# GiorgiaAuroraAdorni/gansformer-reproducibility-challenge

Measured on NVIDIA H100. Metric: images/sec @256^2 synth (GANsformer generator forward, K=16 latents, 12 attention layers, batch 32/GPU), higher is better.
Workload: dtype tf32 (fp32 storage; wgmma tf32 attention and stride-1 3x3 convolutions (own kernels), TF32 cuDNN up-convolutions; value_fp32_convs = the same with fp32 cuDNN convolutions)

## Files before the change

gansformer-reproducibility-challenge_b200/_lib.py:

```python
from __future__ import annotations

import ctypes
from ctypes import c_int, c_int32, c_size_t, c_void_p, c_char_p, POINTER, byref
from typing import Optional

from ._build import LIB_PATH, build_extension

GF_OK = 0
NORM = {None: 0, "none": 0, "layer": 1, "instance": 2, "batch": 3}
INTEGRATION = {"mul": 0, "add": 1, "both": 2}
FLAG_FP32_EXACT = 1
FLAG_CENTROIDS_IN = 2
FLAG_TABLES_READY = 4
FLAG_IMG2LTNT = 8
FLAG_CENTROIDS_INIT = 16
PATH_NAMES = {0: "none", 1: "simt_fp32", 2: "wgmma_tf32"}

WEIGHT_FIELDS = ("wq", "bq", "wpq", "wk", "bk", "wpk", "wv", "bv", "wo", "bo", "pos_latent",
                 "wq2", "bq2", "wpq2", "wk2", "bk2", "wpk2", "wv2", "bv2", "wkc", "wcq", "wi2l", "bi2l")

EXPORTS = ("gf_attn_abi_version", "gf_last_error", "gf_attn_last_path", "gf_attn_folded_floats",
           "gf_attn_fold_weights", "gf_attn_workspace_bytes", "gf_attn_prologue", "gf_attn_simplex_fwd",
           "gf_attn_duplex_fwd", "gf_attn_norm_stats", "gf_attn_launch_count",
           "gf_attn_simplex_fwd_ex", "gf_attn_duplex_fwd_ex", "gf_attn_prologue_ex", "gf_attn_simplex_bwd", "gf_attn_last_centroid_path", "gf_attn_debug_layout",
           "gf_attn_prologue_batch", "gf_attn_tc_eligible", "gf_attn_simplex_bwd_ex", "gf_attn_dropout_mask",
           "gf_attn_centroid_stats", "gf_attn_centroid_bwd")
OPS_EXPORTS = ("gf_chan_scale_nhwc", "gf_blur_up_nhwc", "gf_upsample2x_nchw", "gf_bias_act_nhwc", "gf_demod_coef", "gf_torgb_nhwc", "gf_fir4_nhwc", "gf_blur_up_phases_nhwc", "gf_torgb_scale_nhwc", "gf_mapping_fwd", "gf_conv3x3_pack_weights", "gf_conv3x3_nhwc_tf32", "gf_demod_coef_batch")


class GfAttnDesc(ctypes.Structure):
    _fields_ = [(n, c_int32) for n in ("B", "H", "W", "C", "k", "D", "heads", "norm", "integration",
                                       "pos_dim", "duplex", "flags")]


class GfAttnWeights(ctypes.Structure):
    _fields_ = [(n, c_void_p) for n in WEIGHT_FIELDS]


class GfAttnPostop(ctypes.Structure):
    _fields_ = [("bias", c_void_p), ("noise", c_void_p), ("strength", c_void_p), ("noise_bstride", ctypes.c_longlong),
                ("act", c_int32), ("gain", ctypes.c_float), ("in_scale", c_void_p), ("post_scale", c_void_p),
                ("in_scale_ld", c_int32), ("post_scale_ld", c_int32),
                ("rgb_w", c_void_p), ("rgb_bias", c_void_p), ("rgb_out", c_void_p),
                ("att_dp", ctypes.c_float), ("dp_salt", ctypes.c_uint32), ("dp_state", c_void_p)]


_lib: Optional[ctypes.CDLL] = None


def load() -> ctypes.CDLL:
    global _lib
    if _lib is not None:
        return _lib
    import os
    alt = os.environ.get("GF_ATTN_LIB")
    if alt:
        lib = ctypes.CDLL(alt)
    else:
        try:
            build_extension()
        except Exception as e:
            if not LIB_PATH.exists():
                raise RuntimeError(f"libgf_attn.so is missing and could not be built: {e}") from e
        lib = ctypes.CDLL(str(LIB_PATH))
    lib.gf_attn_abi_version.restype = c_int
    lib.gf_last_error.restype = c_char_p
    lib.gf_attn_last_path.restype = c_int
    lib.gf_attn_folded_floats.argtypes = [POINTER(GfAttnDesc), POINTER(c_size_t)]
    lib.gf_attn_workspace_bytes.argtypes = [POINTER(GfAttnDesc), POINTER(c_size_t)]
    lib.gf_attn_fold_weights.argtypes = [POINTER(GfAttnDesc), POINTER(GfAttnWeights), c_void_p, c_void_p]
    lib.gf_attn_prologue.argtypes = [POINTER(GfAttnDesc), c_void_p, c_void_p, c_void_p, c_void_p]
    lib.gf_attn_simplex_fwd.argtypes = [POINTER(GfAttnDesc), c_void_p, c_void_p, c_void_p, c_void_p, c_void_p]
    lib.gf_attn_duplex_fwd.argtypes = [POINTER(GfAttnDesc), c_void_p, c_void_p, c_void_p, c_void_p, c_void_p,
                                       c_void_p, c_void_p, c_void_p]
    lib.gf_attn_norm_stats.argtypes = [POINTER(GfAttnDesc), c_void_p, c_void_p, c_void_p]
    lib.gf_attn_debug_layout.argtypes = [POINTER(GfAttnDesc), POINTER(ctypes.c_longlong), c_int]
    lib.gf_attn_prologue_ex.argtypes = [POINTER(GfAttnDesc), c_void_p, c_void_p, c_void_p, POINTER(GfAttnPostop), c_void_p]
    lib.gf_attn_simplex_fwd_ex.argtypes = [POINTER(GfAttnDesc), c_void_p, c_void_p, c_void_p, c_void_p, POINTER(GfAttnPostop), c_void_p]
    lib.gf_attn_duplex_fwd_ex.argtypes = [POINTER(GfAttnDesc), c_void_p, c_void_p, c_void_p, c_void_p, c_void_p,
                                          c_void_p, c_void_p, POINTER(GfAttnPostop), c_void_p]
    lib.gf_attn_prologue_batch.argtypes = [c_int, c_void_p, c_void_p, c_void_p, c_void_p, c_void_p, c_void_p]
    lib.gf_attn_simplex_bwd.argtypes = [POINTER(GfAttnDesc)] + [c_void_p] * 11
    lib.gf_attn_simplex_bwd_ex.argtypes = [POINTER(GfAttnDesc)] + [c_void_p] * 10 + [ctypes.c_float, ctypes.c_uint32, c_void_p, c_void_p, c_void_p]
    lib.gf_attn_dropout_mask.argtypes = [POINTER(GfAttnDesc), ctypes.c_float, ctypes.c_uint32, c_void_p, c_void_p, c_void_p]
    lib.gf_attn_centroid_stats.argtypes = [POINTER(GfAttnDesc)] + [c_void_p] * 8
    lib.gf_attn_centroid_bwd.argtypes = [POINTER(GfAttnDesc)] + [c_void_p] * 10
    lib.gf_chan_scale_nhwc.argtypes = [c_void_p, c_void_p, c_int, c_void_p, c_int, c_int, c_int, c_void_p]
    lib.gf_blur_up_nhwc.argtypes = [c_void_p, c_void_p, c_void_p, c_int, c_int, c_int, c_int, ctypes.c_float, c_void_p]
    lib.gf_upsample2x_nchw.argtypes = [c_void_p, c_void_p, c_void_p, c_int, c_int, c_int, c_int, c_void_p]
    lib.gf_bias_act_nhwc.argtypes = [c_void_p, c_void_p, c_void_p, c_void_p, c_void_p, ctypes.c_longlong, c_int, c_int, c_int,
                                     c_int, ctypes.c_float, c_void_p]
    lib.gf_demod_coef.argtypes = [c_void_p, c_int, c_void_p, c_void_p, c_int, c_int, c_int, ctypes.c_float, c_void_p]
    lib.gf_blur_up_phases_nhwc.argtypes = [c_void_p, c_void_p, c_void_p, c_void_p, c_void_p, c_void_p, c_int, c_int, c_int, c_int,
                                           ctypes.c_float, c_void_p]
    lib.gf_fir4_nhwc.argtypes = [c_void_p, c_void_p, c_int, c_int, c_int, c_int, c_int, ctypes.c_float, c_void_p]
    lib.gf_torgb_scale_nhwc.argtypes = [c_void_p, c_void_p, c_void_p, c_int, c_void_p, ctypes.c_float, c_void_p, c_void_p, c_int, c_void_p,
                                        c_int, c_int, c_int, c_void_p]
    lib.gf_mapping_fwd.argtypes = [c_void_p, c_void_p, c_void_p, c_void_p, ctypes.c_float, c_void_p, c_int, c_int, c_int, c_int, c_void_p]
    lib.gf_conv3x3_pack_weights.argtypes = [c_void_p, c_void_p, c_int, c_int, ctypes.c_float, c_void_p]
    lib.gf_conv3x3_nhwc_tf32.argtypes = [c_void_p, c_void_p, c_void_p, c_int, c_int, c_int, c_int, c_int, c_void_p]
    lib.gf_demod_coef_batch.argtypes = [c_void_p, c_int, c_int, ctypes.c_float, c_void_p]
    lib.gf_torgb_nhwc.argtypes = [c_void_p, c_void_p, c_void_p, c_int, c_void_p, ctypes.c_float, c_void_p, c_int, c_int, c_int, c_void_p]
    for name in OPS_EXPORTS:
        getattr(lib, name).restype = c_int
    for name in EXPORTS:
        fn = getattr(lib, name)
        if name not in ("gf_last_error", "gf_attn_launch_count"):
            fn.restype = c_int
    lib.gf_attn_launch_count.restype = ctypes.c_longlong
    lib.gf_attn_tc_eligible.argtypes = [POINTER(GfAttnDesc)]
    if lib.gf_attn_abi_version() != 2:
        raise RuntimeError("libgf_attn.so ABI version mismatch")
    _lib = lib
    return lib


class GfDemodJob(ctypes.Structure):
    _fields_ = [("styles", c_void_p), ("wsq", c_void_p), ("d", c_void_p), ("s_ld", ctypes.c_int32), ("O", ctypes.c_int32),
                ("I", ctypes.c_int32), ("pad_", ctypes.c_int32)]


DEMOD_MAX_JOBS = 32


def check(rc: int, what: str) -> None:
    if rc != GF_OK:
        msg = load().gf_last_error().decode("utf-8", "replace")
        raise RuntimeError(f"{what} failed (gf_status {rc}): {msg}")


def make_desc(B, H, W, C, k, D, *, heads=1, norm="layer", integration="mul", pos_dim=0, duplex=False, flags=0) -> GfAttnDesc:
    if norm not in NORM:
        raise ValueError(f"unknown norm {norm!r}")
    if integration not in INTEGRATION:
        raise ValueError(f"unknown integration {integration!r}")
    return GfAttnDesc(B, H, W, C, k, D, heads, NORM[norm], INTEGRATION[integration], pos_dim, int(duplex), flags)


def folded_floats(desc: GfAttnDesc) -> int:
    out = c_size_t(0)
    check(load().gf_attn_folded_floats(byref(desc), byref(out)), "gf_attn_folded_floats")
    return out.value


def workspace_bytes(desc: GfAttnDesc) -> int:
    out = c_size_t(0)
    check(load().gf_attn_workspace_bytes(byref(desc), byref(out)), "gf_attn_workspace_bytes")
    return out.value


def launch_count() -> int:
    return int(load().gf_attn_launch_count())


def last_centroid_path() -> str:
    return PATH_NAMES.get(load().gf_attn_last_centroid_path(), "?")


def last_path() -> str:
    return PATH_NAMES.get(load().gf_attn_last_path(), "?")
```

gansformer-reproducibility-challenge_b200/csrc/gf_conv.cu:

```cuda
#include <stdlib.h>
#include <string.h>
#include "gf_common.cuh"
#include "gf_tc_common.cuh"
#include "../../include/gf_ops.h"

namespace gf {
namespace cv {

using namespace tc;

constexpr int PH = 8, PW = 16;
constexpr int BK = 32;
constexpr int A_ROWS = (PH + 2) * PW;
constexpr int A_BYTES = A_ROWS * BK * 4;
constexpr int NUM_THREADS = 288;
constexpr int MAX_A = 3, MAX_W = 8;

struct Bars {
  uint64_t full_a[MAX_A], empty_a[MAX_A], full_w[MAX_W], empty_w[MAX_W];
};

struct Params {
  int B, H, W, Cin, Cout;
  int tiles_h, tiles_w, tiles_n;
// ... 39 lines not shown
    if (lane == 0) {
      int sa = 0, sw = 0; uint32_t pa = 0, pw_ = 0;
      for (long long t = blockIdx.x; t < P.total_tiles; t += gridDim.x) {
        int nt, pw, ph, b;
        decode(t, nt, pw, ph, b);
        const int h0 = ph * PH, w0 = pw * PW, n0 = nt * BN;
        for (int c0 = 0; c0 < P.Cin; c0 += BK) {
          for (int dx = 0; dx < 3; ++dx) {
            mbar_wait(smem_u32(&bars->empty_a[sa]), pa ^ 1u);
            const uint32_t fa = smem_u32(&bars->full_a[sa]);
            mbar_expect_tx(fa, (uint32_t)A_BYTES);
            tma_load_4d(s_a + (uint32_t)sa * A_BYTES, &tmX, fa, c0, w0 + dx - 1, h0 - 1, b);
            if (++sa == P.na) { sa = 0; pa ^= 1u; }
            for (int dy = 0; dy < 3; ++dy) {
              mbar_wait(smem_u32(&bars->empty_w[sw]), pw_ ^ 1u);
              const uint32_t fw = smem_u32(&bars->full_w[sw]);
              mbar_expect_tx(fw, (uint32_t)W_BYTES);
              tma_load_2d(s_w + (uint32_t)sw * W_BYTES, &tmW, fw, c0, (dy * 3 + dx) * P.Cout + n0);
              if (++sw == P.nw) { sw = 0; pw_ ^= 1u; }
            }
          }
        }
      }
    }
    return;
  }

  const int wg = warp >> 2;
  const int gid = lane >> 2, qd = lane & 3;
  const int rA = wg * 64 + (warp & 3) * 16 + gid;
  const bool leader = (warp & 3) == 0 && lane == 0;
  int sa = 0, sw = 0; uint32_t pa = 0, pw_ = 0;
  for (long long t = blockIdx.x; t < P.total_tiles; t += gridDim.x) {
    int nt, pw, ph, b;
    decode(t, nt, pw, ph, b);
    float acc[BN / 2];
    int prev_w = -1, prev_a = -1;
#pragma unroll 1
    for (int c0 = 0; c0 < P.Cin; c0 += BK) {
#pragma unroll 1
      for (int dx = 0; dx < 3; ++dx) {
        mbar_wait(smem_u32(&bars->full_a[sa]), pa);
        const uint32_t a_view = s_a + (uint32_t)sa * A_BYTES + wg * 64 * 128;
#pragma unroll
        for (int dy = 0; dy < 3; ++dy) {
          mbar_wait(smem_u32(&bars->full_w[sw]), pw_);
          const uint64_t da = gmma_desc(a_view + dy * PW * 128, 1024, LAYOUT_SW128);
          const uint64_t db = gmma_desc(s_w + (uint32_t)sw * W_BYTES, 1024, LAYOUT_SW128);
          const uint32_t acc0 = (c0 | dx | dy) ? 1u : 0u;
          wgmma_fence();
#pragma unroll
          for (int kk = 0; kk < 4; ++kk) wgmma_ss<BN>(acc, da + kk * 2, db + kk * 2, (acc0 | kk) ? 1u : 0u);
          wgmma_commit();
          wgmma_wait<1>();
          if (prev_w >= 0) {
            named_bar_sync(1 + wg, 128);
            if (leader) {
              mbar_arrive(smem_u32(&bars->empty_w[prev_w]));
              if (prev_a >= 0) mbar_arrive(smem_u32(&bars->empty_a[prev_a]));
            }
          }
          prev_w = sw;
          prev_a = dy == 2 ? sa : -1;
          if (++sw == P.nw) { sw = 0; pw_ ^= 1u; }
        }
        if (++sa == P.na) { sa = 0; pa ^= 1u; }
      }
    }
    wgmma_wait<0>();
    fence_regs<BN / 2>(acc);
    named_bar_sync(1 + wg, 128);
    if (leader) {
      mbar_arrive(smem_u32(&bars->empty_w[prev_w]));
      mbar_arrive(smem_u32(&bars->empty_a[prev_a]));
    }
#pragma unroll
    for (int i = 0; i < 2; ++i) {
      const int r = rA + 8 * i;
      const int h = ph * PH + (r >> 4), w = pw * PW + (r & 15);
      float* yrow = y + (((size_t)b * P.H + h) * P.W + w) * P.Cout + nt * BN + 2 * qd;
#pragma unroll
      for (int j = 0; j < BN / 8; ++j)
        *reinterpret_cast<float2*>(yrow + 8 * j) = make_float2(acc[4 * j + 2 * i] * P.alpha, acc[4 * j + 2 * i + 1] * P.alpha);
    }
  }
}

static int make_map_nhwc(CUtensorMap* m, const void* base, int B, int H, int W, int C, int box_c, int box_w, int box_h) {
  EncodeTiledFn enc = get_encode();
  if (!enc) { set_error("cuTensorMapEncodeTiled entry point not available"); return GF_ERR_CUDA; }
  cuuint64_t dims[4] = {(cuuint64_t)C, (cuuint64_t)W, (cuuint64_t)H, (cuuint64_t)B};
  cuuint64_t strides[3] = {(cuuint64_t)C * 4, (cuuint64_t)W * C * 4, (cuuint64_t)H * W * C * 4};
  cuuint32_t box[4] = {(cuuint32_t)box_c, (cuuint32_t)box_w, (cuuint32_t)box_h, 1};
  cuuint32_t estr[4] = {1, 1, 1, 1};
  CUresult r = enc(m, CU_TENSOR_MAP_DATA_TYPE_FLOAT32, 4, const_cast<void*>(base), dims, strides, box, estr, CU_TENSOR_MAP_INTERLEAVE_NONE,
                   CU_TENSOR_MAP_SWIZZLE_128B, CU_TENSOR_MAP_L2_PROMOTION_L2_128B, CU_TENSOR_MAP_FLOAT_OOB_FILL_NONE);
  if (r != CUDA_SUCCESS) { set_error("cuTensorMapEncodeTiled (NHWC 4-D) failed with CUresult %d (B=%d H=%d W=%d C=%d)", (int)r, B, H, W, C); return GF_ERR_CUDA; }
  return GF_OK;
}

template <int BN>
static int launch_bn(const float* x, const float* wt, float* y, int B, int H, int W, int Cin, int Cout, cudaStream_t st) {
  constexpr int W_BYTES = BN * BK * 4;
  CUtensorMap tmX, tmW;
  int rc;
  if ((rc = make_map_nhwc(&tmX, x, B, H, W, Cin, BK, PW, PH + 2))) return rc;
  if ((rc = make_map(&tmW, wt, (uint64_t)9 * Cout, (uint64_t)Cin, BN, BK, CU_TENSOR_MAP_SWIZZLE_128B))) return rc;
  Params P;
  P.B = B; P.H = H; P.W = W; P.Cin = Cin; P.Cout = Cout;
  P.tiles_h = H / PH; P.tiles_w = W / PW; P.tiles_n = Cout / BN;
  P.total_tiles = (long long)B * P.tiles_h * P.tiles_w * P.tiles_n;
  const int avail = device_smem_optin() - (int)sizeof(Bars) - 1024;
  P.na = MAX_A;
  P.nw = (avail - P.na * A_BYTES) / W_BYTES;
  if (P.nw > MAX_W) P.nw = MAX_W;
  if (P.nw < 2) { set_error("conv3x3: shared memory too small"); return GF_ERR_UNSUPPORTED; }
  P.alpha = 1.000352220f;
  const int smem_bytes = P.na * A_BYTES + P.nw * W_BYTES + (int)sizeof(Bars) + 1024;
  GF_CUDA_OK(cudaFuncSetAttribute(conv3x3_tc_kernel<BN>, cudaFuncAttributeMaxDynamicSharedMemorySize, smem_bytes));
  long long grid = device_sms();
  if (grid > P.total_tiles) grid = P.total_tiles;
  conv3x3_tc_kernel<BN><<<(unsigned)grid, NUM_THREADS, smem_bytes, st>>>(tmX, tmW, y, P);
  GF_LAUNCH_OK();
  return GF_OK;
}

static int launch(const float* x, const float* wt, float* y, int B, int H, int W, int Cin, int Cout, cudaStream_t st) {
  if (Cout % 256 == 0) return launch_bn<256>(x, wt, y, B, H, W, Cin, Cout, st);
  if (Cout % 128 == 0) return launch_bn<128>(x, wt, y, B, H, W, Cin, Cout, st);
  return launch_bn<64>(x, wt, y, B, H, W, Cin, Cout, st);
}

__global__ void pack_weights_kernel(const float* __restrict__ w, float* __restrict__ wt, int Cout, int Cin, float scale) {
  const size_t total = (size_t)9 * Cout * Cin;
  for (size_t i = blockIdx.x * (size_t)blockDim.x + threadIdx.x; i < total; i += (size_t)gridDim.x * blockDim.x) {
    const int ci = (int)(i % Cin);
    const int o = (int)((i / Cin) % Cout);
    const int tap = (int)(i / ((size_t)Cin * Cout));
    wt[i] = round_tf32_rn(w[((size_t)o * Cin + ci) * 9 + tap] * scale);
  }
}

}
}

using namespace gf;

extern "C" int gf_conv3x3_pack_weights(const float* w, float* wt, int Cout, int Cin, float scale, void* stream) {
  if (!w || !wt || Cout <= 0 || Cin <= 0) { set_error("gf_conv3x3_pack_weights: bad arguments"); return GF_ERR_INVALID; }
  const size_t total = (size_t)9 * Cout * Cin;
  size_t blocks = (total + 255) / 256;
  if (blocks > (size_t)num_sms() * 16) blocks = (size_t)num_sms() * 16;
  cv::pack_weights_kernel<<<(unsigned)blocks, 256, 0, (cudaStream_t)stream>>>(w, wt, Cout, Cin, scale);
  GF_LAUNCH_OK();
  return GF_OK;
}

extern "C" int gf_conv3x3_nhwc_tf32(const float* x, const float* wt, float* y, int B, int H, int W, int Cin, int Cout, void* stream) {
  if (!x || !wt || !y) { set_error("gf_conv3x3_nhwc_tf32: null pointer"); return GF_ERR_INVALID; }
  if (B <= 0 || H <= 0 || W <= 0 || H % cv::PH || W % cv::PW || Cin % cv::BK || Cout % 64 || Cin <= 0 || Cout <= 0) {
    set_error("gf_conv3x3_nhwc_tf32: needs positive sizes, H %% 8 == 0, W %% 16 == 0, Cin %% 32 == 0, Cout %% 64 == 0 (got B=%d H=%d W=%d Cin=%d Cout=%d)", B, H, W, Cin, Cout);
    return GF_ERR_UNSUPPORTED;
  }
  if (((uintptr_t)x & 15) || ((uintptr_t)wt & 15) || ((uintptr_t)y & 15)) { set_error("gf_conv3x3_nhwc_tf32: pointers must be 16-byte aligned"); return GF_ERR_INVALID; }
  int rc;
  if ((rc = check_device())) return rc;
  return cv::launch(x, wt, y, B, H, W, Cin, Cout, (cudaStream_t)stream);
}
```

gansformer-reproducibility-challenge_b200/networks.py:

```python
from __future__ import annotations

import math
import os
from typing import List, Optional

import numpy as np
import torch
import torch.nn.functional as F
from torch import nn

from .attention import BipartiteAttention, _Plan, prologue_batch, tc_eligible
from . import ops
from ._state import weights_epoch, bump_weights_epoch
from .ops import fir_filter

SQRT2 = math.sqrt(2.0)


def _inference(*params) -> bool:
    return not (torch.is_grad_enabled() and any(p.requires_grad for p in params))


CACHE_BYPASS = False


def _cached(module: nn.Module, key: str, params, fn):
    if CACHE_BYPASS:
        with torch.no_grad():
            return fn()
    ver = (weights_epoch(),) + tuple((p.data_ptr(), p._version, str(p.device), p.dtype) for p in params)
    store = module.__dict__.setdefault("_icache", {})
    ent = store.get(key)
    if ent is None or ent[0] != ver:
        with torch.no_grad():
            ent = (ver, fn())
        store[key] = ent
    return ent[1]


RUNTIME_KEYS = ("_icache", "_graphs", "_side_stream", "_copy_stream")


def drop_runtime_state(module: nn.Module) -> nn.Module:
    for m in module.modules():
        for key in [k for k in m.__dict__ if k in RUNTIME_KEYS or (isinstance(k, tuple) and k and k[0] == "_staging")]:
            del m.__dict__[key]
        if isinstance(m, BipartiteAttention):
            m._plan = _Plan()
    return module


def nf(res: int, fmap_base: int = 16384, fmap_max: int = 512) -> int:
    return int(min(fmap_base // (2 ** (int(math.log2(res)) - 1)), fmap_max))


def modulated_conv2d(x: torch.Tensor, weight: torch.Tensor, styles: torch.Tensor, *, demodulate: bool = True,
                     up: int = 1, f: Optional[torch.Tensor] = None, w_eff: Optional[torch.Tensor] = None,
                     wsq: Optional[torch.Tensor] = None, prescaled: bool = False, defer_demod: bool = False,
                     d: Optional[torch.Tensor] = None, phases=None, wt_packed: Optional[torch.Tensor] = None):
    O, I, kh, kw = weight.shape
    if w_eff is None:
        w_eff = weight * (1.0 / math.sqrt(I * kh * kw))
        if up != 1:
            w_eff = w_eff.transpose(0, 1)
    if demodulate and d is None:
        if wsq is None:
            wsq = (weight * (1.0 / math.sqrt(I * kh * kw))).square().sum(dim=[2, 3])
        d = ops.demod_coef(styles, wsq)
    if not prescaled:
        x = ops.chan_scale(x, styles)
    if up == 1:
        if wt_packed is not None:
            x = ops.conv3x3_native(x, wt_packed)
        else:
            x = F.conv2d(x, w_eff, padding=kh // 2)
        if defer_demod:
            return x, d
        if d is not None:
            x = ops.chan_scale(x, d)
    elif phases is not None and ops._use_cuda(x, d) and O % 4 == 0 and not os.environ.get("GF_NO_PHASES"):
        x = ops.upconv_blur_phases(x, phases, scale=d, gain=4.0)
    else:
        x = F.conv_transpose2d(x, w_eff, stride=2)
        x = ops.blur_up(x, f, scale=d, gain=4.0)
    return x


class FullyConnected(nn.Module):
    def __init__(self, in_features: int, out_features: int, bias_init: float = 0.0, lr_mul: float = 1.0, act: str = "linear"):
        super().__init__()
        self.weight = nn.Parameter(torch.randn(out_features, in_features) / lr_mul)
        self.bias = nn.Parameter(torch.full((out_features,), float(bias_init)))
        self.wgain = lr_mul / math.sqrt(in_features)
        self.bgain = lr_mul
        self.act = act

    def effective(self):
        g = SQRT2 if self.act == "lrelu" else 1.0
        return (self.weight * (self.wgain * g)).t().contiguous(), self.bias * (self.bgain * g)

    def forward(self, x):
        if _inference(self.weight, self.bias):
            wt, b = _cached(self, "eff", (self.weight, self.bias), self.effective)
            y = torch.addmm(b, x.reshape(-1, x.shape[-1]), wt).reshape(*x.shape[:-1], wt.shape[1])
            return F.leaky_relu(y, 0.2) if self.act == "lrelu" else y
        x = F.linear(x, self.weight * self.wgain, self.bias * self.bgain)
        return F.leaky_relu(x, 0.2) * SQRT2 if self.act == "lrelu" else x


class MappingNetwork(nn.Module):

    def __init__(self, latent_dim: int, components_num: int, num_layers: int = 8, lr_mul: float = 0.01, ltnt2ltnt: bool = False,
                 integration: str = "mul", norm: Optional[str] = "layer", exact_fp32: bool = False):
        super().__init__()
        self.latent_dim, self.components_num = latent_dim, components_num
        self.local = nn.ModuleList([FullyConnected(latent_dim, latent_dim, lr_mul=lr_mul, act="lrelu") for _ in range(num_layers)])
        self.glob = nn.ModuleList([FullyConnected(latent_dim, latent_dim, lr_mul=lr_mul, act="lrelu") for _ in range(num_layers)])
        self.register_buffer("w_avg", torch.zeros(2, latent_dim))
        self.self_att = None
        if ltnt2ltnt and components_num > 1:
            self.self_att = nn.ModuleList([BipartiteAttention(latent_dim, latent_dim, components_num, pos_dim=latent_dim, use_pos=False,
                                                              integration=integration, norm=norm, exact_fp32=exact_fp32)
                                           for _ in range(num_layers)])

    def forward(self, z: torch.Tensor, truncation_psi: float = 1.0) -> torch.Tensor:
        k = self.components_num
        if z.dim() != 3 or z.shape[1] != k + 1 or z.shape[2] != self.latent_dim:
            raise ValueError(f"z must be [B, {k + 1}, {self.latent_dim}], got {tuple(z.shape)}")
        params = [t for fc in list(self.local) + list(self.glob) for t in (fc.weight, fc.bias)]
        if (self.self_att is None and z.is_cuda and z.dtype == torch.float32 and _inference(*params) and self.latent_dim <= 128
                and len(self.local) * self.latent_dim ** 2 * 8 <= 200 * 1024 and not os.environ.get("GF_NO_MAPPING_KERNEL")):
            def stack():
                wl, bl = zip(*[fc.effective() for fc in self.local])
                wg, bg = zip(*[fc.effective() for fc in self.glob])
                return (torch.stack([torch.stack(wl), torch.stack(wg)]).contiguous(), torch.stack([torch.stack(bl), torch.stack(bg)]).contiguous())
            w_eff, b_eff = _cached(self, "stack", params, stack)
            return ops.mapping_fwd(z, w_eff, b_eff, self.w_avg, float(truncation_psi), k)
        z = z * torch.rsqrt(z.square().mean(dim=2, keepdim=True) + 1e-8)
        loc, glo = z[:, :k], z[:, k:]
        for i, fc in enumerate(self.local):
            loc = fc(loc)
            if self.self_att is not None:
                loc = loc.contiguous()
                loc, _, _ = self.self_att[i](loc.reshape(loc.shape[0], k, 1, self.latent_dim), loc)
                loc = loc.reshape(-1, k, self.latent_dim)
        for fc in self.glob:
            glo = fc(glo)
        if truncation_psi != 1.0:
            loc = self.w_avg[0].lerp(loc, truncation_psi)
            glo = self.w_avg[1].lerp(glo, truncation_psi)
        return torch.cat([loc, glo], dim=1)


class SynthesisLayer(nn.Module):

    def __init__(self, in_ch: int, out_ch: int, w_dim: int, resolution: int, up: bool, components_num: int,
                 use_attention: bool, attn_kwargs: dict):
        super().__init__()
        self.resolution, self.up = resolution, up
        self.affine = FullyConnected(w_dim, in_ch, bias_init=1.0)
        self.weight = nn.Parameter(torch.randn(out_ch, in_ch, 3, 3))
        self.bias = nn.Parameter(torch.zeros(out_ch))
        self.register_buffer("noise_const", torch.randn(resolution, resolution))
        self.noise_strength = nn.Parameter(torch.zeros([]))
        self.register_buffer("fir", fir_filter())
        self.attention = BipartiteAttention(out_ch, w_dim, components_num, **attn_kwargs) if use_attention else None

    def _conv_weights(self):
        O, I, kh, kw = self.weight.shape
        w = self.weight * (1.0 / math.sqrt(I * kh * kw))
        wsq = w.square().sum(dim=[2, 3])
        phases = ops.upconv_phase_weights(w) if self.up else None
        packed = None
        if not self.up and w.is_cuda and kh == 3 and I % 32 == 0 and O % 64 == 0:
            packed = ops.conv3x3_pack(w)
        if self.up:
            w = w.transpose(0, 1)
        return w.contiguous(memory_format=torch.channels_last), wsq.contiguous(), phases, packed

    def fusable(self, x) -> bool:
        a = self.attention
        return (a is not None and x.is_cuda and a.norm in ("layer", None, "none")
                and _inference(self.weight, self.bias, self.noise_strength, *a.parameters()))

    def forward(self, x, w_glob, y, noise_mode="const", centroids=None, return_att=False, styles=None,
                prescaled=False, post_scale=None, prepared=None, rgb=None, centroids_init=None, demod=None):
        if styles is None:
            styles = self.affine(w_glob)
        w_eff = wsq = phases = packed = None
        if _inference(self.weight) and x.is_cuda:
            w_eff, wsq, phases, packed = _cached(self, "conv", (self.weight,), self._conv_weights)
            if packed is not None and not (torch.backends.cudnn.allow_tf32 and x.dtype == torch.float32 and x.shape[2] % 8 == 0
                                           and x.shape[3] % 16 == 0 and not os.environ.get("GF_CUDNN_CONV")):
                packed = None
        fused = self.fusable(x)
        in_scale = None
        if prepared is not None and not fused:
            raise RuntimeError("internal: prepared prologue for a layer that does not take the fused path")
        if fused and not self.up:
            x, in_scale = modulated_conv2d(x, self.weight, styles, up=1, f=self.fir, w_eff=w_eff, wsq=wsq,
                                           prescaled=prescaled, defer_demod=True, d=prepared[1] if prepared is not None else demod,
                                           wt_packed=packed)
        else:
            x = modulated_conv2d(x, self.weight, styles, up=2 if self.up else 1, f=self.fir, w_eff=w_eff, wsq=wsq,
                                 prescaled=prescaled, phases=phases, wt_packed=None if self.up else packed, d=demod)
        if noise_mode == "const":
            noise = self.noise_const
        elif noise_mode == "random":
            noise = torch.randn(x.shape[0], 1, self.resolution, self.resolution, device=x.device, dtype=x.dtype)
        else:
            noise = None
        att = None
        if self.attention is not None:
            xl = x.permute(0, 2, 3, 1)
            if not xl.is_contiguous():
                xl = xl.contiguous()
            if fused:
                post = dict(bias=self.bias, noise=noise, strength=self.noise_strength, act="lrelu", gain=SQRT2,
                            in_scale=in_scale, post_scale=post_scale)
                if rgb is not None:
                    post.update(rgb)
                post.update(self.attention.dropout_postop(x.device))
                if prepared is not None and prepared[0] is not None:
                    torch.cuda.current_stream(x.device).wait_event(prepared[0])
                xo, att, centroids = self.attention(xl, y, centroids=centroids, return_att=return_att, postop=post,
                                                    stage="token" if prepared is not None else "all",
                                                    need_centroids=self.attention.iterative,
                                                    centroids_init=centroids_init)
                return xo.permute(0, 3, 1, 2), att, centroids
            xo, att, centroids = self.attention(xl, y, centroids=centroids, return_att=return_att, centroids_init=centroids_init)
            x = xo.permute(0, 3, 1, 2)
        x = ops.bias_act(x, self.bias, "lrelu", noise=noise, strength=self.noise_strength)
        if post_scale is not None:
            x = ops.chan_scale(x, post_scale)
        return x, att, centroids


class ToRGB(nn.Module):
    def __init__(self, in_ch: int, w_dim: int, img_channels: int = 3):
        super().__init__()
        self.affine = FullyConnected(w_dim, in_ch, bias_init=1.0)
        self.weight = nn.Parameter(torch.randn(img_channels, in_ch, 1, 1))
        self.bias = nn.Parameter(torch.zeros(img_channels))

    def forward(self, x, w_glob, styles=None, next_styles=None):
        if styles is None:
            styles = self.affine(w_glob)
        return ops.torgb(x, self.weight, styles, self.bias, next_styles=next_styles)


class SynthesisNetwork(nn.Module):

    def __init__(self, resolution: int, latent_dim: int, components_num: int, fmap_base: int = 16384, fmap_max: int = 512,
                 g_start_res: int = 8, g_end_res: Optional[int] = None, transformer: bool = True, attn_kwargs: Optional[dict] = None):
        super().__init__()
        assert resolution >= 4 and resolution & (resolution - 1) == 0
        self.resolution, self.components_num = resolution, components_num
        g_end_res = resolution if g_end_res is None else g_end_res
        self.block_resolutions = [2 ** i for i in range(2, int(math.log2(resolution)) + 1)]
        attn_kwargs = dict(attn_kwargs or {})
        self.const = nn.Parameter(torch.randn(nf(4, fmap_base, fmap_max), 4, 4))
        self.layers = nn.ModuleList()
        self.torgbs = nn.ModuleList()
        self.layer_res: List[int] = []
        self.iterative = bool(attn_kwargs.get("iterative", False)) and bool(attn_kwargs.get("kmeans", False))
        for res in self.block_resolutions:
            out_ch = nf(res, fmap_base, fmap_max)
            use_att = transformer and components_num > 0 and g_start_res <= res <= g_end_res
            if res > 4:
                in_ch = nf(res // 2, fmap_base, fmap_max)
                self.layers.append(SynthesisLayer(in_ch, out_ch, latent_dim, res, True, components_num, use_att, attn_kwargs))
                self.layer_res.append(res)
            self.layers.append(SynthesisLayer(out_ch, out_ch, latent_dim, res, False, components_num, use_att, attn_kwargs))
            self.layer_res.append(res)
            self.torgbs.append(ToRGB(out_ch, latent_dim))
        self.register_buffer("fir", fir_filter())
        self.num_attention_layers = sum(1 for l in self.layers if l.attention is not None)

    def forward(self, ws: torch.Tensor, noise_mode: str = "const", return_att: bool = False, return_features: bool = False):
        k = self.components_num
        B = ws.shape[0]
        y = ws[:, :k].contiguous()
        w_glob = ws[:, k]
        x = self.const[None].expand(B, -1, -1, -1).contiguous(memory_format=torch.channels_last)
        mods = list(self.layers) + list(self.torgbs)
        aff = [m.affine for m in mods]
        aff_params = [t for a in aff for t in (a.weight, a.bias)]
        styles_all = [None] * len(mods)
# ... 196 lines not shown
```

gansformer-reproducibility-challenge_b200/ops.py:

```python
from __future__ import annotations

import ctypes
import math
from typing import Optional

import torch
import torch.nn.functional as F

from . import _lib

SQRT2 = math.sqrt(2.0)


def _use_cuda(*tensors) -> bool:
    ts = [t for t in tensors if t is not None]
    if not all(t.is_cuda and t.dtype == torch.float32 for t in ts):
        return False
    return not (torch.is_grad_enabled() and any(t.requires_grad for t in ts))


def _stream(dev):
    return ctypes.c_void_p(torch.cuda.current_stream(dev).cuda_stream)


# ... 198 lines not shown
    total = sum(w_.shape[0] for _, w_ in pairs)
    d_all = torch.empty((B * total,), dtype=torch.float32, device=dev)
    jobs = (_lib.GfDemodJob * len(pairs))()
    outs, keep, off = [], [], 0
    for i, (s_, w_) in enumerate(pairs):
        if s_.shape[0] != B or s_.shape[1] != w_.shape[1]:
            raise ValueError("demod_coef_batch: styles [B, I] / wsq [O, I] mismatch")
        sr, ld = _rows(s_)
        wc = w_.contiguous()
        O, I = wc.shape
        d = d_all[off:off + B * O].view(B, O)
        off += B * O
        jobs[i].styles, jobs[i].wsq, jobs[i].d = sr.data_ptr(), wc.data_ptr(), d.data_ptr()
        jobs[i].s_ld, jobs[i].O, jobs[i].I = ld, O, I
        outs.append(d)
        keep += [sr, wc]
    with torch.cuda.device(dev):
        _lib.check(_lib.load().gf_demod_coef_batch(ctypes.cast(jobs, ctypes.c_void_p), len(pairs), B, float(eps), _stream(dev)),
                   "gf_demod_coef_batch")
    return outs


def torgb(x: torch.Tensor, weight: torch.Tensor, styles: torch.Tensor, bias: Optional[torch.Tensor],
          next_styles: Optional[torch.Tensor] = None):
    O, I = weight.shape[:2]
    wscale = 1.0 / math.sqrt(I)
    if _use_cuda(x, weight, styles, bias, next_styles) and O == 3 and I % 4 == 0 and I <= 512:
        xv = _nhwc_view(x)
        B, H, W, C = xv.shape
        y = torch.empty((B, O, H, W), device=x.device, dtype=torch.float32)
        sr, ld = _rows(styles)
        wv = weight.reshape(O, I).contiguous()
        xs = s2 = None
        ld2 = 0
        if next_styles is not None:
            s2, ld2 = _rows(next_styles)
            xs = torch.empty_like(xv)
        with torch.cuda.device(x.device):
            _lib.check(_lib.load().gf_torgb_scale_nhwc(xv.data_ptr(), wv.data_ptr(), sr.data_ptr(), ld,
                                                       bias.data_ptr() if bias is not None else None, ctypes.c_float(wscale),
                                                       y.data_ptr(), None if s2 is None else s2.data_ptr(), ld2,
                                                       None if xs is None else xs.data_ptr(), B, H * W, C, _stream(x.device)),
                       "gf_torgb_scale_nhwc")
        return y if next_styles is None else (y, xs.permute(0, 3, 1, 2))
    wm = weight.reshape(1, O, I).to(x.dtype) * styles[:, None, :].to(x.dtype) * wscale
    B, C, H, W = x.shape
    xl = x.permute(0, 2, 3, 1).reshape(B, H * W, C)
    rgb = torch.matmul(xl, wm.transpose(1, 2))
    if bias is not None:
        rgb = rgb + bias.to(x.dtype)
    rgb = rgb.transpose(1, 2).reshape(B, O, H, W)
    return rgb if next_styles is None else (rgb, x * next_styles[:, :, None, None].to(x.dtype))


def mapping_fwd(z: torch.Tensor, w_eff: torch.Tensor, b_eff: torch.Tensor, w_avg: Optional[torch.Tensor], psi: float, k: int) -> torch.Tensor:
    B, kp1, D = z.shape
    L = w_eff.shape[1]
    out = torch.empty_like(z)
    wa = w_avg.contiguous() if (w_avg is not None and psi != 1.0) else None
    with torch.cuda.device(z.device):
        _lib.check(_lib.load().gf_mapping_fwd(z.contiguous().data_ptr(), w_eff.data_ptr(), b_eff.data_ptr(), wa.data_ptr() if wa is not None else None,
                                              float(psi), out.data_ptr(), B, k, D, L, _stream(z.device)), "gf_mapping_fwd")
    return out


def conv3x3_pack(weight: torch.Tensor, scale: float = 1.0) -> torch.Tensor:
    O, I = weight.shape[:2]
    wt = torch.empty((9, O, I), dtype=torch.float32, device=weight.device)
    with torch.cuda.device(weight.device):
        _lib.check(_lib.load().gf_conv3x3_pack_weights(weight.detach().contiguous().data_ptr(), wt.data_ptr(), O, I, ctypes.c_float(scale),
                                                       _stream(weight.device)), "gf_conv3x3_pack_weights")
    return wt


def conv3x3_native(x: torch.Tensor, wt: torch.Tensor) -> torch.Tensor:
    xv = _nhwc_view(x)
    B, H, W, I = xv.shape
    O = wt.shape[1]
    y = torch.empty((B, H, W, O), dtype=torch.float32, device=x.device)
    with torch.cuda.device(x.device):
        _lib.check(_lib.load().gf_conv3x3_nhwc_tf32(xv.data_ptr(), wt.data_ptr(), y.data_ptr(), B, H, W, I, O, _stream(x.device)),
                   "gf_conv3x3_nhwc_tf32")
    return y.permute(0, 3, 1, 2)
```

include/gf_ops.h:

```cpp
#ifndef GF_OPS_H_
#define GF_OPS_H_

#include <stddef.h>
#include <stdint.h>

#ifdef __cplusplus
extern "C" {
#endif

int gf_chan_scale_nhwc(const float* x, const float* s, int s_ld, float* y, int B, int HW, int C, void* stream);

int gf_blur_up_nhwc(const float* x, float* y, const float* scale, int B, int Hout, int Wout, int C, float gain, void* stream);

int gf_blur_up_phases_nhwc(const float* p00, const float* p01, const float* p10, const float* p11, float* y, const float* scale,
                           int B, int Hout, int Wout, int C, float gain, void* stream);

int gf_fir4_nhwc(const float* x, float* y, int B, int Hin, int Win, int C, int pad, float gain, void* stream);

int gf_upsample2x_nchw(const float* x, const float* add, float* y, int B, int C, int H, int W, void* stream);

int gf_bias_act_nhwc(const float* x, float* y, const float* bias, const float* noise, const float* strength,
                     long long noise_bstride, int B, int HW, int C, int act, float gain, void* stream);

int gf_demod_coef(const float* styles, int s_ld, const float* wsq, float* d, int B, int O, int I, float eps, void* stream);

#define GF_DEMOD_MAX_JOBS 32
typedef struct gf_demod_job {
  const float* styles;
  const float* wsq;
  float* d;
  int32_t s_ld, O, I, pad_;
} gf_demod_job;
int gf_demod_coef_batch(const gf_demod_job* jobs, int n, int B, float eps, void* stream);

int gf_torgb_nhwc(const float* x, const float* w, const float* styles, int s_ld, const float* bias, float wscale, float* y,
                  int B, int HW, int C, void* stream);

int gf_torgb_scale_nhwc(const float* x, const float* w, const float* styles, int s_ld, const float* bias, float wscale, float* y,
                        const float* s2, int s2_ld, float* xs_out, int B, int HW, int C, void* stream);

int gf_mapping_fwd(const float* z, const float* w, const float* b, const float* w_avg, float psi, float* out,
                   int B, int k, int D, int L, void* stream);

int gf_conv3x3_pack_weights(const float* w, float* wt, int Cout, int Cin, float scale, void* stream);
int gf_conv3x3_nhwc_tf32(const float* x, const float* wt, float* y, int B, int H, int W, int Cin, int Cout, void* stream);

#ifdef __cplusplus
}
#endif
#endif
```

Measured before the change: 1969.

## Fuse 3x3 transposed up-convolution with blur into a wgmma TF32 kernel

Adds a warp-specialized TMA plus wgmma kernel that computes the stride-2 transposed 3x3 convolution as four output phases. The 4x4 FIR blur and demodulation scale are applied in the epilogue, with halo rows carried in shared memory between row steps. This replaces the cuDNN up-convolution plus separate blur/phase kernels for up layers at resolution at least 256, which removes an intermediate tensor round trip through global memory. The trade-offs are a complex pipeline, heavy shared-memory use with one block per SM, and a serial epilogue that may limit throughput.

```diff
diff --git a/gansformer-reproducibility-challenge_b200/_lib.py b/gansformer-reproducibility-challenge_b200/_lib.py
--- a/gansformer-reproducibility-challenge_b200/_lib.py
+++ b/gansformer-reproducibility-challenge_b200/_lib.py
@@ -25,7 +25,7 @@
            "gf_attn_simplex_fwd_ex", "gf_attn_duplex_fwd_ex", "gf_attn_prologue_ex", "gf_attn_simplex_bwd", "gf_attn_last_centroid_path", "gf_attn_debug_layout",
            "gf_attn_prologue_batch", "gf_attn_tc_eligible", "gf_attn_simplex_bwd_ex", "gf_attn_dropout_mask",
            "gf_attn_centroid_stats", "gf_attn_centroid_bwd")
-OPS_EXPORTS = ("gf_chan_scale_nhwc", "gf_blur_up_nhwc", "gf_upsample2x_nchw", "gf_bias_act_nhwc", "gf_demod_coef", "gf_torgb_nhwc", "gf_fir4_nhwc", "gf_blur_up_phases_nhwc", "gf_torgb_scale_nhwc", "gf_mapping_fwd", "gf_conv3x3_pack_weights", "gf_conv3x3_nhwc_tf32", "gf_demod_coef_batch")
+OPS_EXPORTS = ("gf_chan_scale_nhwc", "gf_blur_up_nhwc", "gf_upsample2x_nchw", "gf_bias_act_nhwc", "gf_demod_coef", "gf_torgb_nhwc", "gf_fir4_nhwc", "gf_blur_up_phases_nhwc", "gf_torgb_scale_nhwc", "gf_mapping_fwd", "gf_conv3x3_pack_weights", "gf_conv3x3_nhwc_tf32", "gf_demod_coef_batch", "gf_upconv3x3_blur_nhwc_tf32")
 
 
 class GfAttnDesc(ctypes.Structure):
@@ -99,6 +99,8 @@
     lib.gf_mapping_fwd.argtypes = [c_void_p, c_void_p, c_void_p, c_void_p, ctypes.c_float, c_void_p, c_int, c_int, c_int, c_int, c_void_p]
     lib.gf_conv3x3_pack_weights.argtypes = [c_void_p, c_void_p, c_int, c_int, ctypes.c_float, c_void_p]
     lib.gf_conv3x3_nhwc_tf32.argtypes = [c_void_p, c_void_p, c_void_p, c_int, c_int, c_int, c_int, c_int, c_void_p]
+    lib.gf_upconv3x3_blur_nhwc_tf32.argtypes = [c_void_p, c_void_p, c_void_p, c_void_p, c_int, c_int, c_int, c_int, c_int, ctypes.c_float,
+                                                 c_void_p]
     lib.gf_demod_coef_batch.argtypes = [c_void_p, c_int, c_int, ctypes.c_float, c_void_p]
     lib.gf_torgb_nhwc.argtypes = [c_void_p, c_void_p, c_void_p, c_int, c_void_p, ctypes.c_float, c_void_p, c_int, c_int, c_int, c_void_p]
     for name in OPS_EXPORTS:
diff --git a/gansformer-reproducibility-challenge_b200/csrc/gf_conv.cu b/gansformer-reproducibility-challenge_b200/csrc/gf_conv.cu
--- a/gansformer-reproducibility-challenge_b200/csrc/gf_conv.cu
+++ b/gansformer-reproducibility-challenge_b200/csrc/gf_conv.cu
@@ -145,6 +145,203 @@
 #pragma unroll
       for (int j = 0; j < BN / 8; ++j)
         *reinterpret_cast<float2*>(yrow + 8 * j) = make_float2(acc[4 * j + 2 * i] * P.alpha, acc[4 * j + 2 * i + 1] * P.alpha);
+    }
+  }
+}
+
+constexpr int U_PC = 16, U_PR = 8;
+constexpr int U_OC = U_PC - 2;
+constexpr int U_BN = 64;
+constexpr int U_A_BYTES = (U_PR + 1) * U_PC * BK * 4;
+constexpr int U_W_BYTES = U_BN * BK * 4;
+constexpr int U_CS = 68;
+constexpr int U_MAX_A = 4, U_MAX_W = 10;
+
+struct UBars {
+  uint64_t full_a[U_MAX_A], empty_a[U_MAX_A], full_w[U_MAX_W], empty_w[U_MAX_W];
+};
+
+struct UParams {
+  int B, H, W, Cin, Cout;
+  int strips, steps, tiles_n;
+  int total_units;
+  int na, nw;
+  float ag;
+  const float* scale;
+};
+
+__device__ constexpr int U_TAP[9] = {0, 6, 3, 2, 1, 8, 7, 5, 4};
+__device__ constexpr int U_PH[9] = {0, 0, 2, 0, 1, 0, 1, 2, 3};
+__device__ constexpr int U_ROW0[9] = {1, 0, 0, 1, 1, 0, 0, 0, 0};
+__device__ constexpr int U_FIRST[9] = {1, 0, 1, 0, 1, 0, 0, 0, 1};
+
+__global__ void __launch_bounds__(NUM_THREADS, 1)
+upconv_blur_tc_kernel(const __grid_constant__ CUtensorMap tmX, const __grid_constant__ CUtensorMap tmW, float* __restrict__ y, const UParams P) {
+  extern __shared__ __align__(1024) uint8_t smem_raw[];
+  uint8_t* smem = smem_raw + ((1024u - (smem_u32(smem_raw) & 1023u)) & 1023u);
+  const uint32_t s_a = smem_u32(smem);
+  const uint32_t s_w = s_a + (uint32_t)P.na * U_A_BYTES;
+  float* carry = reinterpret_cast<float*>(smem + (size_t)P.na * U_A_BYTES + (size_t)P.nw * U_W_BYTES);
+  float* stage = carry + 4 * 2 * U_PC * U_CS;
+  UBars* bars = reinterpret_cast<UBars*>(stage + U_PR * U_PC * U_CS);
+  const int warp = __shfl_sync(0xffffffffu, (int)(threadIdx.x >> 5), 0);
+  const int lane = threadIdx.x & 31;
+
+  if (warp == 8 && lane == 0) {
+    prefetch_tmap(&tmX); prefetch_tmap(&tmW);
+    for (int i = 0; i < P.na; ++i) { mbar_init(smem_u32(&bars->full_a[i]), 1); mbar_init(smem_u32(&bars->empty_a[i]), 2); }
+    for (int i = 0; i < P.nw; ++i) { mbar_init(smem_u32(&bars->full_w[i]), 1); mbar_init(smem_u32(&bars->empty_w[i]), 2); }
+    fence_barrier_init();
+  }
+  __syncthreads();
+
+  auto decode = [&](int u, int& nt, int& st, int& b) {
+    nt = u % P.tiles_n; u /= P.tiles_n;
+    st = u % P.strips; b = u / P.strips;
+  };
+
+  if (warp == 8) {
+    if (lane == 0) {
+      int sa = 0, sw = 0; uint32_t pa = 0, pw_ = 0;
+      for (int u = blockIdx.x; u < P.total_units; u += gridDim.x) {
+        int nt, st, b;
+        decode(u, nt, st, b);
+        const int j0 = st * U_OC, n0 = nt * U_BN;
+        for (int s = 0; s < P.steps; ++s) {
+          for (int c0 = 0; c0 < P.Cin; c0 += BK) {
+            for (int t = 0; t < 9; ++t) {
+              if (t == 0 || t == 3) {
+                mbar_wait(smem_u32(&bars->empty_a[sa]), pa ^ 1u);
+                const uint32_t fa = smem_u32(&bars->full_a[sa]);
+                mbar_expect_tx(fa, (uint32_t)U_A_BYTES);
+                tma_load_4d(s_a + (uint32_t)sa * U_A_BYTES, &tmX, fa, c0, j0 - (t == 3), s * U_PR - 1, b);
+                if (++sa == P.na) { sa = 0; pa ^= 1u; }
+              }
+              mbar_wait(smem_u32(&bars->empty_w[sw]), pw_ ^ 1u);
+              const uint32_t fw = smem_u32(&bars->full_w[sw]);
+              mbar_expect_tx(fw, (uint32_t)U_W_BYTES);
+              tma_load_2d(s_w + (uint32_t)sw * U_W_BYTES, &tmW, fw, c0, U_TAP[t] * P.Cout + n0);
+              if (++sw == P.nw) { sw = 0; pw_ ^= 1u; }
+            }
+          }
+        }
+      }
+    }
+    return;
+  }
+
+  const int wg = warp >> 2;
+  const int gid = lane >> 2, qd = lane & 3;
+  const bool leader = (warp & 3) == 0 && lane == 0;
+  const int cp = lane & 7, cg = lane >> 3;
+  int sa = 0, sw = 0; uint32_t pa = 0, pw_ = 0;
+  for (int u = blockIdx.x; u < P.total_units; u += gridDim.x) {
+    int nt, st, b;
+    decode(u, nt, st, b);
+    const int j0 = st * U_OC, n0 = nt * U_BN;
+    for (int s = 0; s < P.steps; ++s) {
+      float acc[4][U_BN / 2];
+      int prev_w = -1, prev_a = -1;
+      uint32_t a_view = 0;
+#pragma unroll 1
+      for (int c0 = 0; c0 < P.Cin; c0 += BK) {
+#pragma unroll
+        for (int t = 0; t < 9; ++t) {
+          if (t == 0 || t == 3) {
+            mbar_wait(smem_u32(&bars->full_a[sa]), pa);
+            a_view = s_a + (uint32_t)sa * U_A_BYTES + wg * 4 * U_PC * 128;
+          }
+          mbar_wait(smem_u32(&bars->full_w[sw]), pw_);
+          const uint64_t da = gmma_desc(a_view + U_ROW0[t] * U_PC * 128, 1024, LAYOUT_SW128);
+          const uint64_t db = gmma_desc(s_w + (uint32_t)sw * U_W_BYTES, 1024, LAYOUT_SW128);
+          const uint32_t acc0 = (c0 > 0 || !U_FIRST[t]) ? 1u : 0u;
+          wgmma_fence();
+#pragma unroll
+          for (int kk = 0; kk < 4; ++kk) wgmma_ss<U_BN>(acc[U_PH[t]], da + kk * 2, db + kk * 2, (acc0 | kk) ? 1u : 0u);
+          wgmma_commit();
+          wgmma_wait<1>();
+          if (prev_w >= 0) {
+            named_bar_sync(1 + wg, 128);
+            if (leader) {
+              mbar_arrive(smem_u32(&bars->empty_w[prev_w]));
+              if (prev_a >= 0) mbar_arrive(smem_u32(&bars->empty_a[prev_a]));
+            }
+          }
+          prev_w = sw;
+          prev_a = (t == 2 || t == 8) ? sa : -1;
+          if (++sw == P.nw) { sw = 0; pw_ ^= 1u; }
+          if (t == 2 || t == 8) { if (++sa == P.na) { sa = 0; pa ^= 1u; } }
+        }
+      }
+      wgmma_wait<0>();
+#pragma unroll
+      for (int ph = 0; ph < 4; ++ph) fence_regs<U_BN / 2>(acc[ph]);
+      named_bar_sync(1 + wg, 128);
+      if (leader) {
+        mbar_arrive(smem_u32(&bars->empty_w[prev_w]));
+        mbar_arrive(smem_u32(&bars->empty_a[prev_a]));
+      }
+
+      const int io = s * U_PR - 2 + warp;
+#pragma unroll
+      for (int sl = 0; sl < U_BN / 16; ++sl) {
+        float* my_row = stage + warp * U_PC * U_CS;
+#pragma unroll
+        for (int ph = 0; ph < 4; ++ph)
+#pragma unroll
+          for (int jj = 0; jj < 2; ++jj)
+#pragma unroll
+            for (int i = 0; i < 2; ++i)
+              *reinterpret_cast<float2*>(my_row + (gid + 8 * i) * U_CS + ph * 16 + jj * 8 + 2 * qd) =
+                  make_float2(acc[ph][4 * (2 * sl + jj) + 2 * i], acc[ph][4 * (2 * sl + jj) + 2 * i + 1]);
+        named_bar_sync(3, 256);
+        if (io >= 0 && io < P.H) {
+          auto row = [&](int r) -> const float* {
+            return (r < 2 ? carry + (sl * 2 + r) * U_PC * U_CS : stage + (r - 2) * U_PC * U_CS) + 2 * cp;
+          };
+          const int ch = n0 + sl * 16 + 2 * cp;
+          const float2 d = __ldg(reinterpret_cast<const float2*>(P.scale + (size_t)b * P.Cout + ch));
+          const float2 f = make_float2(P.ag * d.x, P.ag * d.y);
+          const int Wo = 2 * P.W;
+#pragma unroll 1
+          for (int p = cg; p < U_OC && j0 + p < P.W; p += 4) {
+            float* y0 = y + (((size_t)b * 2 * P.H + 2 * io) * Wo + 2 * (j0 + p)) * P.Cout + ch;
+#pragma unroll 1
+            for (int cb = 0; cb < 2; ++cb) {
+              const int oA = cb ? 0 : 16, oB = cb ? U_CS + 16 : 0, oC = cb ? U_CS : U_CS + 16, oD = cb ? 2 * U_CS + 16 : U_CS;
+              float2 e, o;
+#pragma unroll
+              for (int v = 0; v < 5; ++v) {
+                const float* base = row(warp + v / 2) + ((v & 1) ? 0 : 32) + p * U_CS;
+                const float2 A = *reinterpret_cast<const float2*>(base + oA), B_ = *reinterpret_cast<const float2*>(base + oB);
+                const float2 C = *reinterpret_cast<const float2*>(base + oC), D = *reinterpret_cast<const float2*>(base + oD);
+                float2 hv;
+                hv.x = ((A.x + 3.f * B_.x) + 3.f * C.x) + D.x;
+                hv.y = ((A.y + 3.f * B_.y) + 3.f * C.y) + D.y;
+                if (v == 0) { e = hv; }
+                else if (v == 1) { e.x += 3.f * hv.x; e.y += 3.f * hv.y; o = hv; }
+                else if (v == 2) { e.x += 3.f * hv.x; e.y += 3.f * hv.y; o.x += 3.f * hv.x; o.y += 3.f * hv.y; }
+                else if (v == 3) { e.x += hv.x; e.y += hv.y; o.x += 3.f * hv.x; o.y += 3.f * hv.y; }
+                else { o.x += hv.x; o.y += hv.y; }
+              }
+              *reinterpret_cast<float2*>(y0 + cb * P.Cout) = make_float2(e.x * 0.015625f * f.x, e.y * 0.015625f * f.y);
+              *reinterpret_cast<float2*>(y0 + (size_t)Wo * P.Cout + cb * P.Cout) = make_float2(o.x * 0.015625f * f.x, o.y * 0.015625f * f.y);
+            }
+          }
+        }
+        named_bar_sync(3, 256);
+        if (warp >= U_PR - 2) {
+          float* crow = carry + (sl * 2 + warp - (U_PR - 2)) * U_PC * U_CS;
+#pragma unroll
+          for (int ph = 0; ph < 4; ++ph)
+#pragma unroll
+            for (int jj = 0; jj < 2; ++jj)
+#pragma unroll
+              for (int i = 0; i < 2; ++i)
+                *reinterpret_cast<float2*>(crow + (gid + 8 * i) * U_CS + ph * 16 + jj * 8 + 2 * qd) =
+                    make_float2(acc[ph][4 * (2 * sl + jj) + 2 * i], acc[ph][4 * (2 * sl + jj) + 2 * i + 1]);
+        }
+      }
     }
   }
 }
@@ -194,6 +391,36 @@
   return launch_bn<64>(x, wt, y, B, H, W, Cin, Cout, st);
 }
 
+static int launch_upconv(const float* x, const float* wt, const float* scale, float* y, int B, int H, int W, int Cin, int Cout,
+                         float gain, cudaStream_t st) {
+  CUtensorMap tmX, tmW;
+  int rc;
+  if ((rc = make_map_nhwc(&tmX, x, B, H, W, Cin, BK, U_PC, U_PR + 1))) return rc;
+  if ((rc = make_map(&tmW, wt, (uint64_t)9 * Cout, (uint64_t)Cin, U_BN, BK, CU_TENSOR_MAP_SWIZZLE_128B))) return rc;
+  UParams P;
+  P.B = B; P.H = H; P.W = W; P.Cin = Cin; P.Cout = Cout;
+  P.strips = (W + U_OC - 1) / U_OC;
+  P.steps = (H + 2 + U_PR - 1) / U_PR;
+  P.tiles_n = Cout / U_BN;
+  const long long units = (long long)B * P.strips * P.tiles_n;
+  if (units > (1ll << 30)) { set_error("upconv3x3_blur: too many work units (%lld)", units); return GF_ERR_UNSUPPORTED; }
+  P.total_units = (int)units;
+  P.ag = 1.000352220f * gain;
+  P.scale = scale;
+  const int fixed = 8 * U_PC * U_CS * 4 + U_PR * U_PC * U_CS * 4 + (int)sizeof(UBars) + 1024;
+  P.na = U_MAX_A;
+  P.nw = (device_smem_optin() - fixed - P.na * U_A_BYTES) / U_W_BYTES;
+  if (P.nw > U_MAX_W) P.nw = U_MAX_W;
+  if (P.nw < 3) { set_error("upconv3x3_blur: shared memory too small"); return GF_ERR_UNSUPPORTED; }
+  const int smem_bytes = fixed + P.na * U_A_BYTES + P.nw * U_W_BYTES;
+  GF_CUDA_OK(cudaFuncSetAttribute(upconv_blur_tc_kernel, cudaFuncAttributeMaxDynamicSharedMemorySize, smem_bytes));
+  long long grid = device_sms();
+  if (grid > P.total_units) grid = P.total_units;
+  upconv_blur_tc_kernel<<<(unsigned)grid, NUM_THREADS, smem_bytes, st>>>(tmX, tmW, y, P);
+  GF_LAUNCH_OK();
+  return GF_OK;
+}
+
 __global__ void pack_weights_kernel(const float* __restrict__ w, float* __restrict__ wt, int Cout, int Cin, float scale) {
   const size_t total = (size_t)9 * Cout * Cin;
   for (size_t i = blockIdx.x * (size_t)blockDim.x + threadIdx.x; i < total; i += (size_t)gridDim.x * blockDim.x) {
@@ -230,3 +457,18 @@
   if ((rc = check_device())) return rc;
   return cv::launch(x, wt, y, B, H, W, Cin, Cout, (cudaStream_t)stream);
 }
+
+extern "C" int gf_upconv3x3_blur_nhwc_tf32(const float* x, const float* wt, const float* scale, float* y, int B, int H, int W, int Cin,
+                                           int Cout, float gain, void* stream) {
+  if (!x || !wt || !scale || !y) { set_error("gf_upconv3x3_blur_nhwc_tf32: null pointer"); return GF_ERR_INVALID; }
+  if (B <= 0 || H <= 0 || W <= 0 || Cin <= 0 || Cout <= 0 || Cin % cv::BK || Cout % cv::U_BN) {
+    set_error("gf_upconv3x3_blur_nhwc_tf32: needs positive sizes, Cin %% 32 == 0, Cout %% 64 == 0 (got B=%d H=%d W=%d Cin=%d Cout=%d)", B, H, W, Cin, Cout);
+    return GF_ERR_UNSUPPORTED;
+  }
+  if (((uintptr_t)x & 15) || ((uintptr_t)wt & 15) || ((uintptr_t)y & 15) || ((uintptr_t)scale & 15)) {
+    set_error("gf_upconv3x3_blur_nhwc_tf32: pointers must be 16-byte aligned"); return GF_ERR_INVALID;
+  }
+  int rc;
+  if ((rc = check_device())) return rc;
+  return cv::launch_upconv(x, wt, scale, y, B, H, W, Cin, Cout, gain, (cudaStream_t)stream);
+}
diff --git a/gansformer-reproducibility-challenge_b200/networks.py b/gansformer-reproducibility-challenge_b200/networks.py
--- a/gansformer-reproducibility-challenge_b200/networks.py
+++ b/gansformer-reproducibility-challenge_b200/networks.py
@@ -20,6 +20,8 @@
 def _inference(*params) -> bool:
     return not (torch.is_grad_enabled() and any(p.requires_grad for p in params))
 
+
+UPCONV_FUSED_MIN_RES = 256
 
 CACHE_BYPASS = False
 
@@ -78,6 +80,8 @@
             return x, d
         if d is not None:
             x = ops.chan_scale(x, d)
+    elif wt_packed is not None and d is not None and ops._use_cuda(x, d):
+        x = ops.upconv_blur_native(x, wt_packed, scale=d, gain=4.0)
     elif phases is not None and ops._use_cuda(x, d) and O % 4 == 0 and not os.environ.get("GF_NO_PHASES"):
         x = ops.upconv_blur_phases(x, phases, scale=d, gain=4.0)
     else:
@@ -172,7 +176,7 @@
         wsq = w.square().sum(dim=[2, 3])
         phases = ops.upconv_phase_weights(w) if self.up else None
         packed = None
-        if not self.up and w.is_cuda and kh == 3 and I % 32 == 0 and O % 64 == 0:
+        if w.is_cuda and kh == 3 and I % 32 == 0 and O % 64 == 0 and (not self.up or self.resolution >= UPCONV_FUSED_MIN_RES):
             packed = ops.conv3x3_pack(w)
         if self.up:
             w = w.transpose(0, 1)
@@ -190,8 +194,9 @@
         w_eff = wsq = phases = packed = None
         if _inference(self.weight) and x.is_cuda:
             w_eff, wsq, phases, packed = _cached(self, "conv", (self.weight,), self._conv_weights)
-            if packed is not None and not (torch.backends.cudnn.allow_tf32 and x.dtype == torch.float32 and x.shape[2] % 8 == 0
-                                           and x.shape[3] % 16 == 0 and not os.environ.get("GF_CUDNN_CONV")):
+            if packed is not None and not (torch.backends.cudnn.allow_tf32 and x.dtype == torch.float32
+                                           and (self.up or (x.shape[2] % 8 == 0 and x.shape[3] % 16 == 0
+                                                            and not os.environ.get("GF_CUDNN_CONV")))):
                 packed = None
         fused = self.fusable(x)
         in_scale = None
@@ -203,7 +208,7 @@
                                            wt_packed=packed)
         else:
             x = modulated_conv2d(x, self.weight, styles, up=2 if self.up else 1, f=self.fir, w_eff=w_eff, wsq=wsq,
-                                 prescaled=prescaled, phases=phases, wt_packed=None if self.up else packed, d=demod)
+                                 prescaled=prescaled, phases=phases, wt_packed=packed, d=demod)
         if noise_mode == "const":
             noise = self.noise_const
         elif noise_mode == "random":
diff --git a/gansformer-reproducibility-challenge_b200/ops.py b/gansformer-reproducibility-challenge_b200/ops.py
--- a/gansformer-reproducibility-challenge_b200/ops.py
+++ b/gansformer-reproducibility-challenge_b200/ops.py
@@ -304,3 +304,15 @@
         _lib.check(_lib.load().gf_conv3x3_nhwc_tf32(xv.data_ptr(), wt.data_ptr(), y.data_ptr(), B, H, W, I, O, _stream(x.device)),
                    "gf_conv3x3_nhwc_tf32")
     return y.permute(0, 3, 1, 2)
+
+
+def upconv_blur_native(x: torch.Tensor, wt: torch.Tensor, scale: torch.Tensor, gain: float = 4.0) -> torch.Tensor:
+    xv = _nhwc_view(x)
+    B, H, W, I = xv.shape
+    O = wt.shape[1]
+    y = torch.empty((B, 2 * H, 2 * W, O), dtype=torch.float32, device=x.device)
+    sc = scale.contiguous()
+    with torch.cuda.device(x.device):
+        _lib.check(_lib.load().gf_upconv3x3_blur_nhwc_tf32(xv.data_ptr(), wt.data_ptr(), sc.data_ptr(), y.data_ptr(),
+                                                           B, H, W, I, O, ctypes.c_float(gain), _stream(x.device)), "gf_upconv3x3_blur_nhwc_tf32")
+    return y.permute(0, 3, 1, 2)
diff --git a/include/gf_ops.h b/include/gf_ops.h
--- a/include/gf_ops.h
+++ b/include/gf_ops.h
@@ -45,6 +45,9 @@
 int gf_conv3x3_pack_weights(const float* w, float* wt, int Cout, int Cin, float scale, void* stream);
 int gf_conv3x3_nhwc_tf32(const float* x, const float* wt, float* y, int B, int H, int W, int Cin, int Cout, void* stream);
 
+int gf_upconv3x3_blur_nhwc_tf32(const float* x, const float* wt, const float* scale, float* y, int B, int H, int W, int Cin, int Cout,
+                                float gain, void* stream);
+
 #ifdef __cplusplus
 }
 #endif
```

New measurement: 2176 (median of 6 runs). +10.5%, better.
